# divortio/divortio-lz4

Hardware: NVIDIA B200
Metric: lz4_block_roundtrip_throughput (higher is better)
Workload: dtype u8

## Files before the change

### divortio-lz4_b200/csrc/api_ctx.inc

```
namespace {

constexpr int kWarpsFresh16 = 7;
constexpr int kWarpsGeneric32 = 3;
constexpr int kWarpsDecode = 8;
constexpr int kJdGroupEvent = 112;
constexpr int kGtabRegions = 5;
constexpr uint32_t kMaxSplitBlocks = 1u << 20;

struct Buf {
    void *p = nullptr;
    size_t cap = 0;
};

class CopyPool {
  public:
    explicit CopyPool(int threads) {
        for (int i = 0; i < threads; ++i) workers_.emplace_back([this] { run(); });
    }
    ~CopyPool() {
        { std::lock_guard<std::mutex> g(m_); stop_ = true; }
        cv_.notify_all();
        for (std::thread &t : workers_) t.join();
    }
    void copy(void *dst, const void *src, size_t n) {
// ... 42 lines not shown
    std::vector<std::thread> workers_;
    std::mutex m_;
    std::condition_variable cv_, cv_done_;
    bool stop_ = false;
    uint64_t gen_ = 0;
    uint8_t *dst_ = nullptr;
    const uint8_t *src_ = nullptr;
    size_t n_ = 0, piece_ = 0, parts_ = 0, done_ = 0;
    std::atomic<size_t> next_{0};
};
constexpr int kSumSlots = 32;
constexpr int kStageSlots = 4;
constexpr size_t kStageBytes = 16u << 20;

}

struct dlz4_ctx {
    int device = 0;
    int sm_count = 0;
    cudaStream_t stream = nullptr, side = nullptr, copy_in = nullptr, copy_out = nullptr;
    cudaStream_t lanes[4] = {};
    uint64_t chunk_bytes = 64ull << 20;
    int n_lanes = 3;
    cudaEvent_t evp[128] = {};
    cudaEvent_t ev0 = nullptr, ev1 = nullptr, ev_side = nullptr, ev_fork = nullptr;
    uint32_t *d_counter = nullptr;
    uint32_t *d_land = nullptr;
    uint32_t *h_one = nullptr;
    uint64_t seg_overlap_min_bytes = 64ull << 20;
    uint32_t *d_hash = nullptr;
    uint64_t *d_total = nullptr;
    int32_t *d_table = nullptr;
    int split = 1;
    int pw = 2;
    int pw_sleep = 200;
    int pw_lead = 7;
    Buf rec;
    uint32_t *d_nrec = nullptr;
    int hybrid = 1;
    int hy_grid = 0;
    int hy_active = 0;
    uint16_t *d_gtabs = nullptr;
    Buf work, comp, seg, out, meta, aux, pin;
    std::string last_error;
    uint64_t frame_pipe_min_bytes = 32ull << 20;
    uint64_t jump_min_bytes = 256ull << 10;
    uint64_t seg_min_bytes = 256ull << 10;
    uint32_t seg_jobs = 0, seg_reruns = 0, seg_rounds = 0;
    uint64_t launches = 0;
    float last_ms = 0.f;
    int64_t k_seg_kib = -1, k_seg_warm_kib = -1, k_seg_unit_kib = -1;
    int k_seg_group = -1, k_seg_no_chase = 0, k_jd_unit_mib = 0, k_jd_serial_scan = 0, k_jd_no_overlap = 0, k_debug = 0;
    CopyPool *pool = nullptr;
    int copy_threads = 0;
    uint8_t *stage[kStageSlots] = {};
    cudaEvent_t stage_ev[kStageSlots] = {};
    bool stage_busy[kStageSlots] = {};
    cudaStream_t sum_stream[kSumSlots] = {};
    uint32_t *h_sum = nullptr;
    int probe = 0;
    cudaEvent_t evq[3] = {};
    const uint8_t *res_in = nullptr, *res_out = nullptr;
    uint64_t res_in_len = 0, res_out_len = 0, res_body_len = 0;
};

namespace {

// ... 123 lines not shown
```

### divortio-lz4_b200/csrc/api_launch.inc

```
int compress_segmented(dlz4_ctx *ctx, const uint8_t *d_work, int64_t start, int64_t total, int64_t B, uint32_t n, bool linked,
                       const int32_t *init_table, uint8_t *d_comp, const uint64_t *d_coff, uint32_t *d_clen, cudaStream_t st,
                       int32_t *final_table = nullptr, const uint32_t *landed = nullptr, int32_t land_origin = 0,
                       uint32_t land_shift = 0);

int launch_compress(dlz4_ctx *ctx, const uint8_t *src, const uint64_t *src_off, const uint32_t *src_len, uint32_t n,
                    uint32_t max_len, const uint8_t *prefix, uint32_t prefix_len, const int32_t *init_table, uint8_t *dst,
                    const uint64_t *dst_off, uint32_t *comp_len, cudaStream_t st, uint32_t *counter = nullptr, bool dense = false) {
    if (n == 0) return DLZ4_OK;
    if (!counter) counter = ctx->d_counter;
    CK(cudaMemsetAsync(counter, 0, sizeof(uint32_t), st));
    if (init_table == nullptr) { prefix = nullptr; prefix_len = 0; }
    if (max_len <= 65536 && prefix_len == 0 && init_table == nullptr && ctx->split && n <= kMaxSplitBlocks) {
        const size_t region = (size_t)(counter - ctx->d_counter) % kGtabRegions;
        const uint64_t rstride = (uint64_t)max_len / 4 + 2;
        const size_t region_bytes = (((size_t)n * rstride * 8) * 9 / 8 + 255) & ~(size_t)255;
        if (ctx->rec.cap < region_bytes * kGtabRegions + 256) {
            CK(cudaDeviceSynchronize());
            CKS(reserve(ctx, ctx->rec, std::max(region_bytes, (size_t)ctx->rec.cap / kGtabRegions) * kGtabRegions));
        }
        const size_t per_region = ((ctx->rec.cap - 256) / kGtabRegions) & ~(size_t)255;
        uint64_t *recs = (uint64_t *)((uint8_t *)ctx->rec.p + region * per_region);
        uint32_t *nrec = ctx->d_nrec + region * (size_t)kMaxSplitBlocks;
        if (ctx->probe) CK(cudaEventRecord(ctx->evq[0], st));
        if (ctx->pw) {
            const int grid = (int)std::min<uint64_t>(n, (uint64_t)ctx->sm_count);
            const uint32_t lead = (uint32_t)ctx->pw_lead, ns = (uint32_t)ctx->pw_sleep;
            const size_t sm = (size_t)kPwChains * kPwChainBytes;
            if (ctx->pw == 2)
                k_parse_pw<2><<<grid, kPwChains * 3 * 32, sm, st>>>(src, src_off, src_len, n, recs, rstride, nrec, counter, lead, ns);
            else
                k_parse_pw<3><<<grid, kPwChains * 4 * 32, sm, st>>>(src, src_off, src_len, n, recs, rstride, nrec, counter, lead, ns);
        } else
        {
            const int grid = (int)std::min<uint64_t>((n + kWarpsFresh16 - 1) / kWarpsFresh16, (uint64_t)ctx->sm_count);
            k_parse_fresh16<kWarpsFresh16><<<grid, kWarpsFresh16 * 32, kWarpsFresh16 * kHashEntries * 2, st>>>(
                src, src_off, src_len, n, recs, rstride, nrec, counter);
        }
        if (ctx->probe) CK(cudaEventRecord(ctx->evq[1], st));
        CK(cudaMemsetAsync(counter, 0, sizeof(uint32_t), st));
        const int egrid = (int)std::min<uint64_t>((n + kWarpsDecode - 1) / kWarpsDecode, (uint64_t)ctx->sm_count * 8);
        k_encode_blocks<kWarpsDecode><<<egrid, kWarpsDecode * 32, 0, st>>>(src, src_off, src_len, n, recs, rstride, nrec, dst, dst_off,
                                                                            comp_len, counter);
        if (ctx->probe) CK(cudaEventRecord(ctx->evq[2], st));
        ctx->launches++;
    } else if (max_len <= 65536 && prefix_len == 0 && init_table == nullptr && ctx->hybrid) {
        const size_t region = (size_t)(counter - ctx->d_counter) % kGtabRegions;
        const int grid = (int)std::min<uint64_t>(dense ? (n + kHyWarps - 1) / kHyWarps : n, (uint64_t)ctx->hy_grid);
        uint32_t active = dense ? (uint32_t)kHyWarps : (uint32_t)std::min<uint64_t>((n + grid - 1) / grid, (uint64_t)kHyWarps);
        if (ctx->hy_active) active = std::min<uint32_t>(active, (uint32_t)ctx->hy_active);
        k_compress_fresh16h<<<grid, kHyWarps * 32, kHySmemBytes, st>>>(
            src, src_off, src_len, n, dst, dst_off, comp_len, counter,
            ctx->d_gtabs + region * (size_t)ctx->hy_grid * kHyGlWarps * kHashEntries, active);
    } else if (max_len <= 4096 && prefix_len > 0 && init_table != nullptr && ctx->hybrid && prefix_len < 0x7FFF0000u) {
        const size_t region = (size_t)(counter - ctx->d_counter) % kGtabRegions;
        const int grid = (int)std::min<uint64_t>(dense ? (n + kHyWarps - 1) / kHyWarps : n, (uint64_t)ctx->hy_grid);
        const uint32_t active = dense ? (uint32_t)kHyWarps : (uint32_t)std::min<uint64_t>((n + grid - 1) / grid, (uint64_t)kHyWarps);
        k_compress_overlay<<<grid, kHyWarps * 32, kHySmemBytes, st>>>(
            src, src_off, src_len, n, prefix, prefix_len, init_table, dst, dst_off, comp_len, counter,
            ctx->d_gtabs + region * (size_t)ctx->hy_grid * kHyGlWarps * kHashEntries, active);
    } else {
        if (max_len > 65536 && prefix_len == 0 && init_table == nullptr && n <= 65536) {
            std::vector<uint64_t> off(n);
            std::vector<uint32_t> len(n);
            CK(cudaMemcpyAsync(off.data(), src_off, (size_t)n * 8, cudaMemcpyDeviceToHost, st));
// ... 57 lines not shown
```

### divortio-lz4_b200/csrc/api_lifecycle.inc

```
int dlz4_init(int device, dlz4_ctx **out) {
    if (!out) return DLZ4_E_INVALID_ARG;
    *out = nullptr;
    dlz4_ctx *ctx = new dlz4_ctx();
    ctx->device = device;
    *out = ctx;
    int count = 0;
    CK(cudaGetDeviceCount(&count));
    if (device < 0 || device >= count) { ctx->last_error = "no such CUDA device"; return DLZ4_E_CUDA; }
    CK(cudaSetDevice(device));
    cudaDeviceProp prop;
    CK(cudaGetDeviceProperties(&prop, device));
    ctx->sm_count = prop.multiProcessorCount;
    CK(cudaStreamCreateWithFlags(&ctx->stream, cudaStreamNonBlocking));
    CK(cudaStreamCreateWithFlags(&ctx->side, cudaStreamNonBlocking));
    CK(cudaStreamCreateWithFlags(&ctx->copy_in, cudaStreamNonBlocking));
    CK(cudaStreamCreateWithFlags(&ctx->copy_out, cudaStreamNonBlocking));
    for (cudaEvent_t &e : ctx->evp) CK(cudaEventCreateWithFlags(&e, cudaEventDisableTiming));
    CK(cudaEventCreate(&ctx->ev0));
    CK(cudaEventCreate(&ctx->ev1));
    for (cudaEvent_t &e : ctx->evq) CK(cudaEventCreate(&e));
    CK(cudaEventCreateWithFlags(&ctx->ev_side, cudaEventDisableTiming));
    CK(cudaEventCreateWithFlags(&ctx->ev_fork, cudaEventDisableTiming));
    for (cudaStream_t &l : ctx->lanes) CK(cudaStreamCreateWithFlags(&l, cudaStreamNonBlocking));
    if (const char *e = getenv("DLZ4_SEG_KIB")) ctx->k_seg_kib = std::max(0, atoi(e));
    if (const char *e = getenv("DLZ4_SEG_WARM_KIB")) ctx->k_seg_warm_kib = std::max(0, atoi(e));
    if (const char *e = getenv("DLZ4_SEG_UNIT_KIB")) ctx->k_seg_unit_kib = std::max(0, atoi(e));
    if (const char *e = getenv("DLZ4_SEG_GROUP")) ctx->k_seg_group = std::max(0, atoi(e));
    ctx->k_seg_no_chase = getenv("DLZ4_SEG_NO_CHASE") != nullptr;
    if (const char *e = getenv("DLZ4_JD_UNIT_MIB")) ctx->k_jd_unit_mib = std::max(1, atoi(e));
    ctx->k_jd_serial_scan = getenv("DLZ4_JD_SERIAL_SCAN") != nullptr;
    ctx->k_jd_no_overlap = getenv("DLZ4_JD_NO_OVERLAP") != nullptr;
    ctx->k_debug = getenv("DLZ4_DEBUG") != nullptr;
    if (const char *e = getenv("DLZ4_CHUNK_MIB")) ctx->chunk_bytes = (uint64_t)std::max(1, atoi(e)) << 20;
    if (const char *e = getenv("DLZ4_LANES")) ctx->n_lanes = std::min(4, std::max(1, atoi(e)));
    if (const char *e = getenv("DLZ4_COPY_THREADS")) ctx->copy_threads = std::min(64, std::max(1, atoi(e)));
    CK(cudaMalloc(&ctx->d_counter, 64));
    CK(cudaMalloc(&ctx->d_land, kLandFlags * 4));
    CK(cudaMallocHost(&ctx->h_one, 64));
    *ctx->h_one = 1u;
    if (const char *e = getenv("DLZ4_SEG_OVERLAP_MIN_MIB")) ctx->seg_overlap_min_bytes = (uint64_t)atoll(e) << 20;
    CK(cudaMalloc(&ctx->d_hash, 64));
    CK(cudaMalloc(&ctx->d_total, 64));
    CK(cudaMalloc(&ctx->d_table, kHashEntries * sizeof(int32_t)));
    if (const char *e = getenv("DLZ4_SEG_MIN_KIB")) ctx->seg_min_bytes = (uint64_t)atoll(e) << 10;
    if (const char *e = getenv("DLZ4_JUMP_MIN_KIB")) ctx->jump_min_bytes = (uint64_t)atoll(e) << 10;
    if (const char *e = getenv("DLZ4_SPLIT")) ctx->split = atoi(e) != 0;
    if (const char *e = getenv("DLZ4_PW")) ctx->pw = std::max(0, std::min(3, atoi(e)));
    if (const char *e = getenv("DLZ4_PW_SLEEP")) ctx->pw_sleep = std::max(0, atoi(e));
    if (const char *e = getenv("DLZ4_PW_LEAD")) ctx->pw_lead = std::max(3, std::min(kPwWin - 1, atoi(e)));
    if (const char *e = getenv("DLZ4_HYBRID")) ctx->hybrid = atoi(e) != 0;
    ctx->hy_grid = ctx->sm_count * kHyCtasPerSm;
    if (const char *e = getenv("DLZ4_HY_ACTIVE")) ctx->hy_active = std::max(0, std::min(kHyWarps, atoi(e)));
    CK(cudaMalloc(&ctx->d_gtabs, (size_t)kGtabRegions * ctx->hy_grid * kHyGlWarps * kHashEntries * 2));
    CK(cudaMalloc(&ctx->d_nrec, (size_t)kGtabRegions * kMaxSplitBlocks * 4));
    CK(cudaFuncSetAttribute(k_parse_fresh16<kWarpsFresh16>, cudaFuncAttributeMaxDynamicSharedMemorySize, kWarpsFresh16 * kHashEntries * 2));
    CK(cudaFuncSetAttribute(k_parse_pw<2>, cudaFuncAttributeMaxDynamicSharedMemorySize, kPwChains * kPwChainBytes));
    CK(cudaFuncSetAttribute(k_parse_pw<3>, cudaFuncAttributeMaxDynamicSharedMemorySize, kPwChains * kPwChainBytes));
    CK(cudaFuncSetAttribute(k_compress_fresh16h, cudaFuncAttributeMaxDynamicSharedMemorySize, kHySmemBytes));
    CK(cudaFuncSetAttribute(k_compress_overlay, cudaFuncAttributeMaxDynamicSharedMemorySize, kHySmemBytes));
    CK(cudaFuncSetAttribute(k_compress_segments, cudaFuncAttributeMaxDynamicSharedMemorySize, kSegSmemBytes));
    CK(cudaFuncSetAttribute(k_compress_generic32<kWarpsGeneric32>, cudaFuncAttributeMaxDynamicSharedMemorySize,
                            kWarpsGeneric32 * (kHashEntries * 4 + kRingBytes)));
    CK(cudaFuncSetAttribute(k_compress_chain, cudaFuncAttributeMaxDynamicSharedMemorySize, kHashEntries * 4 + kRingBytes));
    return DLZ4_OK;
}

void dlz4_shutdown(dlz4_ctx *ctx) {
    if (!ctx) return;
    cudaSetDevice(ctx->device);
    if (ctx->stream) cudaStreamSynchronize(ctx->stream);
    if (ctx->side) cudaStreamSynchronize(ctx->side);
    for (Buf *b : {&ctx->work, &ctx->comp, &ctx->seg, &ctx->out, &ctx->meta, &ctx->aux})
        if (b->p) cudaFree(b->p);
    if (ctx->pin.p) cudaFreeHost(ctx->pin.p);
    if (ctx->d_counter) cudaFree(ctx->d_counter);
    if (ctx->d_land) cudaFree(ctx->d_land);
    if (ctx->h_one) cudaFreeHost(ctx->h_one);
    if (ctx->d_hash) cudaFree(ctx->d_hash);
    if (ctx->d_total) cudaFree(ctx->d_total);
    if (ctx->d_table) cudaFree(ctx->d_table);
    if (ctx->d_gtabs) cudaFree(ctx->d_gtabs);
    if (ctx->d_nrec) cudaFree(ctx->d_nrec);
    if (ctx->rec.p) cudaFree(ctx->rec.p);
    delete ctx->pool;
    for (cudaStream_t s : ctx->sum_stream) if (s) { cudaStreamSynchronize(s); cudaStreamDestroy(s); }
    if (ctx->h_sum) cudaFreeHost(ctx->h_sum);
    for (int i = 0; i < kStageSlots; ++i) {
        if (ctx->stage[i]) cudaFreeHost(ctx->stage[i]);
        if (ctx->stage_ev[i]) cudaEventDestroy(ctx->stage_ev[i]);
    }
// ... 88 lines not shown
```

### divortio-lz4_b200/csrc/dlz4_pw.cuh

```cuda
#pragma once

namespace dlz4 {

constexpr int kPwChains = 6;
constexpr int kPwWin = 14;
constexpr int kPwRingBytes = kPwWin * 32 * 12;
constexpr int kPwCtl = 64;
constexpr int kPwChainBytes = kHashEntries * 2 + kPwRingBytes + kPwCtl;
constexpr uint32_t kPwRingSmc = 160u;
constexpr uint32_t kPwDone = 0x80000000u, kPwSparse = 0x40000000u;
constexpr bool kPwPrefetch = true;
#ifndef DLZ4_PW_CAP
#define DLZ4_PW_CAP 32
#endif
constexpr uint32_t kPwCap = DLZ4_PW_CAP;

struct PwCtl {
    volatile uint32_t w_pos;
    volatile uint32_t block;
};

__device__ __forceinline__ void pw_bar(uint32_t id, uint32_t nthreads) {
    asm volatile("bar.sync %0, %1;" ::"r"(id), "r"(nthreads) : "memory");
}
__device__ __forceinline__ uint32_t pw_lds(const uint32_t *p) {
    uint32_t v;
    asm volatile("ld.volatile.shared.u32 %0, [%1];" : "=r"(v) : "r"((uint32_t)__cvta_generic_to_shared(p)) : "memory");
    return v;
}
__device__ __forceinline__ void pw_sts(uint32_t *p, const uint32_t v) {
    asm volatile("st.volatile.shared.u32 [%0], %1;" ::"r"((uint32_t)__cvta_generic_to_shared(p)), "r"(v) : "memory");
}
__device__ __forceinline__ void pw_prefetch(const void *p) { asm volatile("prefetch.global.L1 [%0];" ::"l"(p)); }
__device__ __forceinline__ uint32_t pw_slot(const uint32_t p) {
    const uint32_t w = p >> 5;
    const uint32_t ws = w - (uint32_t)kPwWin * ((w * 74899u) >> 20);
    return ws * 96u + (p & 31u);
}
__device__ __forceinline__ uint32_t pw_resolve(const uint32_t ml, const uint32_t lane, uint32_t &exitp) {
    uint32_t n = ml == kPwCap ? 255u : lane + (ml ? ml : 1u);
    uint32_t m = 1u << lane;
#pragma unroll
    for (int r = 0; r < 5; ++r) {
        const uint32_t mj = __shfl_sync(FULL, m, n), nj = __shfl_sync(FULL, n, n);
        if (n < 32u) { m |= mj; n = nj; }
    }
    exitp = n;
    return m;
}

__device__ __forceinline__ uint32_t pw_extend(const uint8_t *__restrict__ base, int32_t s0, int32_t m0, int32_t eb,
                                              int32_t matchLimit, uint32_t lane) {
    const int32_t back = s0 - m0;
    auto round4 = [&](int32_t e0, uint32_t &res) -> bool {
        const int32_t q = s0 + e0 + 4 * (int32_t)lane;
        int32_t nv = matchLimit - q;
        nv = nv > 4 ? 4 : nv;
        int32_t eq = 0;
        if (nv > 0) {
            const uint32_t x = ld32u(base + q) ^ ld32u(base + q - back);
            const int32_t e = x ? ((__ffs(x) - 1) >> 3) : 4;
            eq = e < nv ? e : nv;
        }
        const uint32_t stop = __ballot_sync(FULL, eq < 4);
        if (!stop) return false;
        const int l = __ffs(stop) - 1;
        res = (uint32_t)(e0 + 4 * l + __shfl_sync(FULL, eq, l));
        return true;
    };
    uint32_t res = 0;
// ... 9 lines not shown
    const uint32_t cmis = (uint32_t)(reinterpret_cast<uintptr_t>(cb) & 15u);
    const uint32_t wsel = cmis >> 2, bsh = (cmis & 3u) * 8u;
    for (;; eb += 2048) {
        uint32_t eqb[4];
#pragma unroll
        for (int u = 0; u < 4; ++u) {
            const int32_t q = s0 + eb + 512 * u + 16 * (int32_t)lane;
            int32_t nv = matchLimit - q;
            nv = nv > 16 ? 16 : nv;
            eqb[u] = 0;
            if (nv > 0) {
                const uint4 a = __ldg(reinterpret_cast<const uint4 *>(base + q));
                const uint4 *cp = reinterpret_cast<const uint4 *>(base + q - back - (int32_t)cmis);
                const uint4 c0 = __ldg(cp), c1 = __ldg(cp + 1);
                uint32_t v[8] = {c0.x, c0.y, c0.z, c0.w, c1.x, c1.y, c1.z, c1.w};
                uint32_t t[5];
#pragma unroll
                for (int i = 0; i < 5; ++i) t[i] = wsel == 0 ? v[i] : wsel == 1 ? v[i + 1] : wsel == 2 ? v[i + 2] : v[i + 3];
                const uint32_t x0 = a.x ^ __funnelshift_r(t[0], t[1], bsh), x1 = a.y ^ __funnelshift_r(t[1], t[2], bsh);
                const uint32_t x2 = a.z ^ __funnelshift_r(t[2], t[3], bsh), x3 = a.w ^ __funnelshift_r(t[3], t[4], bsh);
                uint32_t e = x0 ? ((uint32_t)(__ffs(x0) - 1) >> 3) : x1 ? 4u + ((uint32_t)(__ffs(x1) - 1) >> 3)
                           : x2 ? 8u + ((uint32_t)(__ffs(x2) - 1) >> 3) : x3 ? 12u + ((uint32_t)(__ffs(x3) - 1) >> 3) : 16u;
                eqb[u] = e < (uint32_t)nv ? e : (uint32_t)nv;
            }
        }
#pragma unroll
        for (int u = 0; u < 4; ++u) {
            const uint32_t stop = __ballot_sync(FULL, eqb[u] < 16u);
            if (stop) { const int l = __ffs(stop) - 1; return (uint32_t)(eb + 512 * u + 16 * l) + __shfl_sync(FULL, eqb[u], l); }
        }
    }
}

constexpr uint32_t kPwGenMask = 0x7FFu;

__device__ __forceinline__ uint32_t pw_count32(const uint4 &q0, const uint4 &q1, const uint4 &q2, const uint32_t cs, const uint32_t *Sw) {
    uint32_t v[12] = {q0.x, q0.y, q0.z, q0.w, q1.x, q1.y, q1.z, q1.w, q2.x, q2.y, q2.z, q2.w};
    const bool s8 = (cs & 8u) != 0, s4 = (cs & 4u) != 0;
#pragma unroll
    for (int k = 0; k < 10; ++k) v[k] = s8 ? v[k + 2] : v[k];
#pragma unroll
    for (int k = 0; k < 9; ++k) v[k] = s4 ? v[k + 1] : v[k];
    const uint32_t csh = (cs & 3u) * 8u;
    uint32_t x[8];
#pragma unroll
    for (int k = 0; k < 8; ++k) x[k] = Sw[k] ^ __funnelshift_r(v[k], v[k + 1], csh);
    const bool h4 = (x[0] | x[1] | x[2] | x[3]) == 0u;
    const uint32_t y0 = h4 ? x[4] : x[0], y1 = h4 ? x[5] : x[1], y2 = h4 ? x[6] : x[2], y3 = h4 ? x[7] : x[3];
    const bool h2 = (y0 | y1) == 0u;
    const uint32_t z0 = h2 ? y2 : y0, z1 = h2 ? y3 : y1;
    const bool h1 = z0 == 0u;
    const uint32_t zz = h1 ? z1 : z0;
    return (h4 ? 16u : 0u) + (h2 ? 8u : 0u) + (h1 ? 4u : 0u) + (zz ? ((uint32_t)(__ffs(zz) - 1) >> 3) : 4u);
}

__device__ __forceinline__ void pw_produce2(const uint8_t *__restrict__ base, const uint32_t k, const bool two, const uint16_t *tab,
                                            uint32_t *ring, const uint32_t lane) {
    const uint32_t pa = 32u * k + lane, pb = pa + 32u;
    const uintptr_t ba = reinterpret_cast<uintptr_t>(base);
    const uint32_t a = (uint32_t)(ba & 3u) + pa;
    const uint32_t *wp = reinterpret_cast<const uint32_t *>(ba & ~(uintptr_t)3) + (a >> 2);
    const uint32_t sh = (a & 3u) * 8u;
    uint32_t w[17];
#pragma unroll
    for (int i = 0; i < 9; ++i) w[i] = __ldg(wp + i);
#pragma unroll
    for (int i = 9; i < 17; ++i) w[i] = two ? __ldg(wp + i) : 0u;
    uint32_t S[16];
#pragma unroll
    for (int i = 0; i < 16; ++i) S[i] = __funnelshift_r(w[i], w[i + 1], sh);
    const uint32_t ha = (S[0] * 2654435761u) >> 18, hb = (S[8] * 2654435761u) >> 18;
    const uint32_t seena = *reinterpret_cast<const volatile uint16_t *>(tab + ha);
    const uint32_t seenb = *reinterpret_cast<const volatile uint16_t *>(tab + hb);
    const bool oka = seena != pa, okb = two && seenb != pb;
    const uint32_t la = oka ? seena : pa, lb = okb ? seenb : pa;
    const uint32_t csa = ((uint32_t)(ba & 15u) + la) & 15u, csb = ((uint32_t)(ba & 15u) + lb) & 15u;
    const uint4 *cqa = reinterpret_cast<const uint4 *>(base + la - csa), *cqb = reinterpret_cast<const uint4 *>(base + lb - csb);
    const uint4 qa0 = __ldg(cqa), qa1 = __ldg(cqa + 1), qa2 = __ldg(cqa + 2);
    const uint4 qb0 = __ldg(cqb), qb1 = __ldg(cqb + 1), qb2 = __ldg(cqb + 2);
    if (kPwPrefetch) {
        pw_prefetch(cqa + 4);
        if (two) { pw_prefetch(cqb + 4); pw_prefetch(wp + 24); }
    }
    const uint32_t va = wide_verify(qa0, qa1, qa2, csa, S), vb = wide_verify(qb0, qb1, qb2, csb, S + 8);
    uint32_t mla = oka ? va : 0u, mlb = okb ? vb : 0u;
    if (kPwCap > 32u && __any_sync(FULL, mla == 32u || mlb == 32u)) {
        if (mla == 32u) {
            const uint4 q3 = __ldg(cqa + 3), q4 = __ldg(cqa + 4);
            mla += two ? pw_count32(qa2, q3, q4, csa, S + 8) : 0u;
        }
        if (mlb == 32u) {
            uint32_t w2[9], S2[8];
#pragma unroll
            for (int i = 0; i < 9; ++i) w2[i] = __ldg(wp + 16 + i);
#pragma unroll
            for (int i = 0; i < 8; ++i) S2[i] = __funnelshift_r(w2[i], w2[i + 1], sh);
            const uint4 q3 = __ldg(cqb + 3), q4 = __ldg(cqb + 4);
            mlb += pw_count32(qb2, q3, q4, csb, S2);
        }
    }
    if (kPwCap > 32u && !two && mla == 32u) {
        uint32_t w2[9], S2[8];
#pragma unroll
        for (int i = 0; i < 9; ++i) w2[i] = __ldg(wp + 8 + i);
#pragma unroll
        for (int i = 0; i < 8; ++i) S2[i] = __funnelshift_r(w2[i], w2[i + 1], sh);
        const uint4 q3 = __ldg(cqa + 3), q4 = __ldg(cqa + 4);
        mla += pw_count32(qa2, q3, q4, csa, S2);
    }
    uint32_t exa, exb;
    const uint32_t pma = pw_resolve(mla, lane, exa), pmb = pw_resolve(mlb, lane, exb);
    const uint32_t loa = ha | (mla << 14) | (((k + 1u) & kPwGenMask) << 21);
    uint32_t *const sa = ring + pw_slot(pa), *const sb = ring + pw_slot(pb);
    pw_sts(sa + 32, seena | (exa << 16));
    pw_sts(sa + 64, pma);
    if (two) {
        pw_sts(sb + 32, seenb | (exb << 16));
        pw_sts(sb + 64, pmb);
    }
    __threadfence_block();
    pw_sts(sa, loa);
    if (two) pw_sts(sb, hb | (mlb << 14) | (((k + 2u) & kPwGenMask) << 21));
}

template <int kNP>
__device__ __forceinline__ void pw_producer(const uint8_t *__restrict__ base, const uint32_t nwin, const uint32_t lead,
                                            const uint32_t j, const uint16_t *tab, uint32_t *ring, PwCtl *ctl, const uint32_t lane,
                                            const uint32_t full_ns) {
    uint32_t k = 2u * j;
    PT_DECL
    for (;;) {
        const uint32_t wpos = ctl->w_pos;
        if (wpos & kPwDone) break;
        if (wpos & kPwSparse) { __nanosleep(1024); PT_MARK(8) continue; }
        const uint32_t wk = wpos >> 5;
        if (k + 1u < wk) k += (wk - k - 2u + 2u * (uint32_t)kNP) / (2u * (uint32_t)kNP) * (2u * (uint32_t)kNP);
        if (k >= nwin) { __nanosleep(1024); PT_MARK(8) continue; }
        if (k + 1u >= wk + lead) { __nanosleep(full_ns); PT_MARK(7) continue; }
        if (kPwPrefetch && lane < 2u && k + 2u * (uint32_t)kNP < nwin) pw_prefetch(base + 32u * (k + 2u * (uint32_t)kNP) + 128u * lane);
        pw_produce2(base, k, k + 1u < nwin, tab, ring, lane);
        PT_MARK(6) PT_COUNT(13, 1)
        k += 2u * (uint32_t)kNP;
    }
    PT_FLUSH
}

__device__ __forceinline__ uint32_t pw_walker(const uint8_t *__restrict__ base, const int32_t len, const uint32_t nwin, uint16_t *tab,
                                              const uint32_t *ring, PwCtl *ctl, uint64_t *__restrict__ rec, const uint32_t lane) {
    const uint32_t lt = (1u << lane) - 1u;
    const int32_t sEnd = len;
    const int32_t mflimit = sEnd - 12;
    const int32_t matchLimit = sEnd - 5;
    const int32_t plimit = (int32_t)(32u * nwin);
    const int32_t rlimit = plimit < mflimit ? plimit : mflimit;
    int32_t sIndex = 0;
    uint32_t smc = 67;
    uint32_t nrec = 0;
    uint32_t pub = 0;
    const SrcFlat S{base};
    Tab16 T{tab, 0};
    uint2 *const rec2 = reinterpret_cast<uint2 *>(rec);
    PT_DECL

    while (sIndex < mflimit) {
        if (smc <= 96u && (sIndex | 31) < rlimit) {
            const uint32_t s = (uint32_t)sIndex, wbase = s & ~31u, sl = s & 31u;
            if (pub != wbase) { pub = wbase; if (lane == 0) ctl->w_pos = wbase; }
            const uint32_t p = wbase + lane;
            const uint32_t want = ((p >> 5) + 1u) & kPwGenMask;
            const uint32_t *slot = ring + pw_slot(p);
            uint32_t ex;
            PT_MARK(14)
            for (;;) {
                ex = pw_lds(slot);
                if (__all_sync(FULL, (ex >> 21) == want)) break;
                __nanosleep(32);
                PT_COUNT(15, 1)
            }
            PT_MARK(1)
            const uint32_t ey = pw_lds(slot + 32);
            const uint32_t PM = pw_lds(slot + 64 + sl - lane), exitp = pw_lds(slot + 32 + sl - lane) >> 16;
            const uint32_t seen = ey & 0xFFFFu;
            const uint32_t h = ex & 0x3FFFu, ml = (ex >> 14) & 127u;
            const uint32_t cur = tab[h];
            const uint32_t claim = __ballot_sync(FULL, ml != 0u);
            const bool probed = (PM >> lane) & 1u;
            const uint32_t tag = p & 0xFFFFu;
            __syncwarp();
            if (probed) tab[h] = (uint16_t)tag;
            __syncwarp();
            const uint32_t r = probed ? (uint32_t)tab[h] : tag;
            const uint32_t bad = __ballot_sync(FULL, probed && (r != tag || cur != seen));
            if (!bad) {
                const uint32_t HM = PM & claim;
                const uint32_t nh = (uint32_t)__popc(HM);
                if (((HM >> lane) & 1u) && ml != kPwCap) rec2[nrec + (uint32_t)__popc(HM & lt)] = rec_pack(p, ml, p - cur);
                if (exitp == 255u) {
                    const uint32_t c = 31u - (uint32_t)__clz(PM);
                    const uint32_t pc = wbase + c, curc = __shfl_sync(FULL, cur, c);
                    const uint32_t mlx = pw_extend(base, (int32_t)pc, (int32_t)curc, (int32_t)kPwCap, matchLimit, lane);
                    if (lane == 0) rec2[nrec + nh - 1u] = rec_pack(pc, mlx, pc - curc);
                    sIndex = (int32_t)(pc + mlx);
                    smc = 67u;
                } else {
                    sIndex = (int32_t)(wbase + exitp);
                    if (HM) smc = 67u + (uint32_t)__popc(PM & ~((2u << (31 - __clz(HM))) - 1u));
                    else smc += (uint32_t)__popc(PM);
                }
                nrec += nh;
                PT_MARK(0) PT_COUNT(9, 1)
                continue;
            }
            const uint32_t inv = (probed && r != tag) ? min(tag, r) : 0xFFFFFFFFu;
            const uint32_t cutpos = __reduce_min_sync(FULL, inv);
// ... 3 lines not shown
            if (probed && lane >= Bl) tab[h] = (uint16_t)cur;
            __syncwarp();
            if (probed && lane < Bl) tab[h] = (uint16_t)tag;
            __syncwarp();
            const uint32_t keep = PM & below, HMk = keep & claim;
            if ((HMk >> lane) & 1u) rec2[nrec + (uint32_t)__popc(HMk & lt)] = rec_pack(p, ml, p - cur);
            nrec += (uint32_t)__popc(HMk);
            if (HMk) smc = 67u + (uint32_t)__popc(keep & ~((2u << (31 - __clz(HMk))) - 1u));
            else smc += (uint32_t)__popc(keep);
            sIndex = (int32_t)(wbase + (uint32_t)__ffs(PM & ~below) - 1u);
            const uint32_t hx = __shfl_sync(FULL, h, (uint32_t)sIndex - wbase);
            const uint32_t cand = tab[hx];
            __syncwarp();
            if (lane == 0) tab[hx] = (uint16_t)sIndex;
            __syncwarp();
            uint32_t mlx = 0;
            if (cand != (uint32_t)sIndex) mlx = pw_extend(base, sIndex, (int32_t)cand, 0, matchLimit, lane);
            if (mlx >= 4u) {
                if (lane == 0) rec2[nrec] = rec_pack((uint32_t)sIndex, mlx, (uint32_t)sIndex - cand);
                ++nrec;
                sIndex += (int32_t)mlx;
                smc = 67u;
            } else {
                sIndex += (int32_t)(smc >> 6);
                ++smc;
            }
            PT_MARK(4) PT_COUNT(10, 1)
            continue;
        }
        if (smc <= kPwRingSmc && sIndex < rlimit) {
            const uint32_t bs = skip_sum(smc);
            const int32_t p = sIndex + (int32_t)(skip_sum(smc + lane) - bs);
            const bool valid = p < rlimit;
            if (pub != (uint32_t)sIndex) { pub = (uint32_t)sIndex; if (lane == 0) ctl->w_pos = pub; }
            const uint32_t *slot = ring + pw_slot((uint32_t)p);
            const uint32_t want = (((uint32_t)p >> 5) + 1u) & kPwGenMask;
            uint32_t lo;
            for (;;) {
                lo = pw_lds(slot);
                const bool ready = !valid || ((lo >> 21) == want);
                if (__all_sync(FULL, ready)) break;
                __nanosleep(20);
            }
            const uint32_t seen = pw_lds(slot + 32) & 0xFFFFu;
            const uint32_t h = lo & 0x3FFFu, ml = (lo >> 14) & 127u;
            const uint32_t cur = tab[h];
            const uint32_t claim = __ballot_sync(FULL, valid && ml != 0u);
            const uint32_t f = claim ? (uint32_t)__ffs(claim) - 1u : 32u;
            const bool active = valid && lane <= f;
            const uint32_t tag = (uint32_t)p & 0xFFFFu;
            __syncwarp();
            if (active) tab[h] = (uint16_t)tag;
            __syncwarp();
            const uint32_t r = active ? (uint32_t)tab[h] : tag;
            const uint32_t bad = __ballot_sync(FULL, active && (r != tag || cur != seen));
            if (!bad) {
                if (claim) {
                    const int32_t pf = sIndex + (int32_t)(skip_sum(smc + f) - bs);
                    const uint32_t curf = __shfl_sync(FULL, cur, f);
                    uint32_t mlf = __shfl_sync(FULL, ml, f);
                    if (mlf == kPwCap) mlf = pw_extend(base, pf, (int32_t)curf, (int32_t)kPwCap, matchLimit, lane);
                    if (lane == 0) rec2[nrec] = rec_pack((uint32_t)pf, mlf, (uint32_t)pf - curf);
                    ++nrec;
                    sIndex = pf + (int32_t)mlf;
                    smc = 67u;
                } else {
                    const uint32_t nv = (uint32_t)__popc(__ballot_sync(FULL, valid));
                    sIndex += (int32_t)(skip_sum(smc + nv) - bs);
                    smc += nv;
                }
                PT_MARK(2) PT_COUNT(11, 1)
                continue;
            }
            const uint32_t inv = (active && r != tag) ? min((uint32_t)p, r) : 0xFFFFFFFFu;
            const uint32_t cutpos = __reduce_min_sync(FULL, inv);
            const uint32_t grp = __ballot_sync(FULL, active && (uint32_t)p <= cutpos);
            const uint32_t stale = __ballot_sync(FULL, active && cur != seen);
            const uint32_t c = min((uint32_t)__popc(grp), stale ? (uint32_t)__ffs(stale) - 1u : 32u);
            if (active && lane >= c) tab[h] = (uint16_t)cur;
            __syncwarp();
            if (active && lane < c) tab[h] = (uint16_t)tag;
            __syncwarp();
            if (c != 0u) {
                sIndex += (int32_t)(skip_sum(smc + c) - bs);
                smc += c;
                PT_MARK(2) PT_COUNT(11, 1)
                continue;
            }
            const uint32_t h0 = __shfl_sync(FULL, h, 0);
            const uint32_t cand = tab[h0];
            __syncwarp();
            if (lane == 0) tab[h0] = (uint16_t)sIndex;
            __syncwarp();
            uint32_t ml0 = 0;
            if (cand != (uint32_t)sIndex) ml0 = pw_extend(base, sIndex, (int32_t)cand, 0, matchLimit, lane);
            if (ml0 >= 4u) {
                if (lane == 0) rec2[nrec] = rec_pack((uint32_t)sIndex, ml0, (uint32_t)sIndex - cand);
                ++nrec;
                sIndex += (int32_t)ml0;
                smc = 67u;
            } else {
                sIndex += (int32_t)(smc >> 6);
                ++smc;
            }
            PT_MARK(2) PT_COUNT(11, 1)
            continue;
        }

        if (smc > kPwRingSmc && sIndex < rlimit) {
            const uint32_t v = (uint32_t)sIndex | kPwSparse;
            if (pub != v) { pub = v; if (lane == 0) ctl->w_pos = pub; }
        }
        const uint32_t base_sum = skip_sum(smc);
        const int32_t p = sIndex + (int32_t)(skip_sum(smc + lane) - base_sum);
        const bool valid = p < mflimit;
        uint32_t seq = 0, h = 0x10000u + lane;
        int32_t cand = -1;
        if (valid) {
            seq = S.ld32(p);
            h = (seq * 2654435761u) >> 18;
            cand = T.get(h);
        }
        const uint32_t same = __match_any_sync(FULL, h);
        const uint32_t prev = same & lt;
        const int j = prev ? 31 - __clz(prev) : (int)lane;
        const int32_t pj = __shfl_sync(FULL, p, j);
        const uint32_t sj = __shfl_sync(FULL, seq, j);
        uint32_t cseq = sj;
        if (prev) cand = pj;
        const bool ok = valid && cand >= 0 && cand != p && (((uint32_t)(p - cand)) >> 16) == 0;
        if (ok && !prev) cseq = S.ld32(cand);
        const bool hit = ok && cseq == seq;
        const uint32_t hits = __ballot_sync(FULL, hit);
        const uint32_t vmask = __ballot_sync(FULL, valid);
        const int hl = __ffs(hits) - 1;
        const uint32_t commit = hits ? ((2u << hl) - 1u) : vmask;
        if (((commit >> lane) & 1u) && ((same & commit) >> lane) == 1u) T.put(h, p);
        __syncwarp();
        if (!hits) {
            if (vmask != FULL) break;
            sIndex += (int32_t)(skip_sum(smc + 32u) - base_sum);
            smc += 32u;
            PT_MARK(3) PT_COUNT(12, 1)
            continue;
        }
        const int32_t s0 = __shfl_sync(FULL, p, hl);
        const int32_t m0 = __shfl_sync(FULL, cand, hl);
        smc = 67;
        const uint32_t ml = pw_extend(base, s0, m0, 4, matchLimit, lane);
        if (lane == 0) rec2[nrec] = rec_pack((uint32_t)s0, ml, (uint32_t)(s0 - m0));
        ++nrec;
        sIndex = s0 + (int32_t)ml;
        PT_MARK(3) PT_COUNT(12, 1)
    }
    PT_MARK(5)
    PT_FLUSH
    return nrec;
}

template <int kNP>
__global__ void __launch_bounds__(kPwChains * (1 + kNP) * 32, 1)
k_parse_pw(const uint8_t *__restrict__ src, const uint64_t *__restrict__ src_off, const uint32_t *__restrict__ src_len,
           uint32_t nblocks, uint64_t *__restrict__ rec_base, uint64_t rec_stride ,
           uint32_t *__restrict__ nrec_out, uint32_t *counter, uint32_t lead,
           uint32_t full_ns ) {
    extern __shared__ __align__(16) uint8_t smem[];
    constexpr uint32_t kRoles = 1 + kNP;
    constexpr uint32_t kTeam = kRoles * 32;
    const uint32_t lane = lane_id(), warp = threadIdx.x >> 5;
    const uint32_t chain = warp / kRoles, role = warp % kRoles;
    const uint32_t tid = threadIdx.x - chain * kTeam;
    uint8_t *const cb = smem + (size_t)chain * kPwChainBytes;
    uint16_t *const tab = reinterpret_cast<uint16_t *>(cb);
    uint32_t *const ring = reinterpret_cast<uint32_t *>(cb + kHashEntries * 2);
    PwCtl *const ctl = reinterpret_cast<PwCtl *>(cb + kHashEntries * 2 + kPwRingBytes);
    const uint32_t bar = 1u + chain;
    uint32_t first = chain * gridDim.x + blockIdx.x;
    const uint32_t qbase = gridDim.x * (uint32_t)kPwChains;
    bool have_first = true;
    for (;;) {
        pw_bar(bar, kTeam);
        if (role == 0 && lane == 0) {
            uint32_t b;
            if (have_first) b = first; else b = qbase + atomicAdd(counter, 1u);
            ctl->block = b < nblocks ? b : 0xFFFFFFFFu;
            ctl->w_pos = 0u;
        }
        have_first = false;
        pw_bar(bar, kTeam);
        const uint32_t b = ctl->block;
        if (b == 0xFFFFFFFFu) return;
        const uint32_t len = src_len[b];
        if (len > 65536u) {
            if (role == 0 && lane == 0) nrec_out[b] = 0xFFFFFFFFu;
            continue;
        }
        {
            uint4 *z = reinterpret_cast<uint4 *>(cb);
            for (uint32_t i = tid; i < (kHashEntries * 2 + kPwRingBytes) / 16; i += kTeam) z[i] = make_uint4(0, 0, 0, 0);
        }
        pw_bar(bar, kTeam);
        const uint8_t *base = src + src_off[b];
        uint64_t *const rec = rec_base + (uint64_t)b * rec_stride;
        const uint32_t nwin = len >= 112u ? (len - 111u) / 32u + 1u : 0u;
        if (role == 0) {
            const uint32_t n = pw_walker(base, (int32_t)len, nwin, tab, ring, ctl, rec, lane);
            if (lane == 0) {
                nrec_out[b] = n;
                ctl->w_pos = kPwDone;
            }
        } else {
            pw_producer<kNP>(base, nwin, lead, role - 1u, tab, ring, ctl, lane, full_ns);
        }
    }
}

}
```

Baseline: 75.24.

## Move parse-walker producer ring from shared memory into tensor memory

```diff
diff --git a/divortio-lz4_b200/csrc/api_ctx.inc b/divortio-lz4_b200/csrc/api_ctx.inc
--- a/divortio-lz4_b200/csrc/api_ctx.inc
+++ b/divortio-lz4_b200/csrc/api_ctx.inc
@@ -98,7 +98,7 @@
     uint64_t *d_total = nullptr;
     int32_t *d_table = nullptr;
     int split = 1;
-    int pw = 2;
+    bool pw = true;
     int pw_sleep = 200;
     int pw_lead = 7;
     Buf rec;
diff --git a/divortio-lz4_b200/csrc/api_launch.inc b/divortio-lz4_b200/csrc/api_launch.inc
--- a/divortio-lz4_b200/csrc/api_launch.inc
+++ b/divortio-lz4_b200/csrc/api_launch.inc
@@ -25,11 +25,7 @@
         if (ctx->pw) {
             const int grid = (int)std::min<uint64_t>(n, (uint64_t)ctx->sm_count);
             const uint32_t lead = (uint32_t)ctx->pw_lead, ns = (uint32_t)ctx->pw_sleep;
-            const size_t sm = (size_t)kPwChains * kPwChainBytes;
-            if (ctx->pw == 2)
-                k_parse_pw<2><<<grid, kPwChains * 3 * 32, sm, st>>>(src, src_off, src_len, n, recs, rstride, nrec, counter, lead, ns);
-            else
-                k_parse_pw<3><<<grid, kPwChains * 4 * 32, sm, st>>>(src, src_off, src_len, n, recs, rstride, nrec, counter, lead, ns);
+            k_parse_pw<<<grid, kPwThreads, kPwSmemBytes, st>>>(src, src_off, src_len, n, recs, rstride, nrec, counter, lead, ns);
         } else
         {
             const int grid = (int)std::min<uint64_t>((n + kWarpsFresh16 - 1) / kWarpsFresh16, (uint64_t)ctx->sm_count);
diff --git a/divortio-lz4_b200/csrc/api_lifecycle.inc b/divortio-lz4_b200/csrc/api_lifecycle.inc
--- a/divortio-lz4_b200/csrc/api_lifecycle.inc
+++ b/divortio-lz4_b200/csrc/api_lifecycle.inc
@@ -45,7 +45,7 @@
     if (const char *e = getenv("DLZ4_SEG_MIN_KIB")) ctx->seg_min_bytes = (uint64_t)atoll(e) << 10;
     if (const char *e = getenv("DLZ4_JUMP_MIN_KIB")) ctx->jump_min_bytes = (uint64_t)atoll(e) << 10;
     if (const char *e = getenv("DLZ4_SPLIT")) ctx->split = atoi(e) != 0;
-    if (const char *e = getenv("DLZ4_PW")) ctx->pw = std::max(0, std::min(3, atoi(e)));
+    if (const char *e = getenv("DLZ4_PW")) ctx->pw = atoi(e) != 0;
     if (const char *e = getenv("DLZ4_PW_SLEEP")) ctx->pw_sleep = std::max(0, atoi(e));
     if (const char *e = getenv("DLZ4_PW_LEAD")) ctx->pw_lead = std::max(3, std::min(kPwWin - 1, atoi(e)));
     if (const char *e = getenv("DLZ4_HYBRID")) ctx->hybrid = atoi(e) != 0;
@@ -54,8 +54,7 @@
     CK(cudaMalloc(&ctx->d_gtabs, (size_t)kGtabRegions * ctx->hy_grid * kHyGlWarps * kHashEntries * 2));
     CK(cudaMalloc(&ctx->d_nrec, (size_t)kGtabRegions * kMaxSplitBlocks * 4));
     CK(cudaFuncSetAttribute(k_parse_fresh16<kWarpsFresh16>, cudaFuncAttributeMaxDynamicSharedMemorySize, kWarpsFresh16 * kHashEntries * 2));
-    CK(cudaFuncSetAttribute(k_parse_pw<2>, cudaFuncAttributeMaxDynamicSharedMemorySize, kPwChains * kPwChainBytes));
-    CK(cudaFuncSetAttribute(k_parse_pw<3>, cudaFuncAttributeMaxDynamicSharedMemorySize, kPwChains * kPwChainBytes));
+    CK(cudaFuncSetAttribute(k_parse_pw, cudaFuncAttributeMaxDynamicSharedMemorySize, kPwSmemBytes));
     CK(cudaFuncSetAttribute(k_compress_fresh16h, cudaFuncAttributeMaxDynamicSharedMemorySize, kHySmemBytes));
     CK(cudaFuncSetAttribute(k_compress_overlay, cudaFuncAttributeMaxDynamicSharedMemorySize, kHySmemBytes));
     CK(cudaFuncSetAttribute(k_compress_segments, cudaFuncAttributeMaxDynamicSharedMemorySize, kSegSmemBytes));
diff --git a/divortio-lz4_b200/csrc/dlz4_pw.cuh b/divortio-lz4_b200/csrc/dlz4_pw.cuh
--- a/divortio-lz4_b200/csrc/dlz4_pw.cuh
+++ b/divortio-lz4_b200/csrc/dlz4_pw.cuh
@@ -2,11 +2,14 @@
 
 namespace dlz4 {
 
-constexpr int kPwChains = 6;
+constexpr int kPwChains = 7;
+constexpr int kPwProducers = 2;
+constexpr int kPwThreads = 8 * (1 + kPwProducers) * 32;
 constexpr int kPwWin = 14;
-constexpr int kPwRingBytes = kPwWin * 32 * 12;
+constexpr uint32_t kPwTmemCols = 128;
 constexpr int kPwCtl = 64;
-constexpr int kPwChainBytes = kHashEntries * 2 + kPwRingBytes + kPwCtl;
+constexpr int kPwChainBytes = kHashEntries * 2 + kPwCtl;
+constexpr int kPwSmemBytes = kPwChains * kPwChainBytes + 16;
 constexpr uint32_t kPwRingSmc = 160u;
 constexpr uint32_t kPwDone = 0x80000000u, kPwSparse = 0x40000000u;
 constexpr bool kPwPrefetch = true;
@@ -16,26 +19,49 @@
 constexpr uint32_t kPwCap = DLZ4_PW_CAP;
 
 struct PwCtl {
-    volatile uint32_t w_pos;
+    uint32_t w_pos;
     volatile uint32_t block;
+    uint32_t ready[kPwWin];
 };
+static_assert(sizeof(PwCtl) <= kPwCtl, "PwCtl");
 
 __device__ __forceinline__ void pw_bar(uint32_t id, uint32_t nthreads) {
     asm volatile("bar.sync %0, %1;" ::"r"(id), "r"(nthreads) : "memory");
 }
-__device__ __forceinline__ uint32_t pw_lds(const uint32_t *p) {
+__device__ __forceinline__ uint32_t pw_ld_acquire(const uint32_t *p) {
     uint32_t v;
-    asm volatile("ld.volatile.shared.u32 %0, [%1];" : "=r"(v) : "r"((uint32_t)__cvta_generic_to_shared(p)) : "memory");
+    asm volatile("ld.acquire.cta.shared.u32 %0, [%1];" : "=r"(v) : "r"((uint32_t)__cvta_generic_to_shared(p)) : "memory");
     return v;
 }
-__device__ __forceinline__ void pw_sts(uint32_t *p, const uint32_t v) {
-    asm volatile("st.volatile.shared.u32 [%0], %1;" ::"r"((uint32_t)__cvta_generic_to_shared(p)), "r"(v) : "memory");
+__device__ __forceinline__ void pw_st_release(uint32_t *p, const uint32_t v) {
+    asm volatile("st.release.cta.shared.u32 [%0], %1;" ::"r"((uint32_t)__cvta_generic_to_shared(p)), "r"(v) : "memory");
+}
+__device__ __forceinline__ void pw_st_release2(uint32_t *p, const uint32_t v0, const uint32_t v1) {
+    asm volatile("st.release.cta.shared.v2.u32 [%0], {%1, %2};" ::"r"((uint32_t)__cvta_generic_to_shared(p)), "r"(v0), "r"(v1) : "memory");
 }
 __device__ __forceinline__ void pw_prefetch(const void *p) { asm volatile("prefetch.global.L1 [%0];" ::"l"(p)); }
-__device__ __forceinline__ uint32_t pw_slot(const uint32_t p) {
-    const uint32_t w = p >> 5;
-    const uint32_t ws = w - (uint32_t)kPwWin * ((w * 74899u) >> 20);
-    return ws * 96u + (p & 31u);
+__device__ __forceinline__ void tm_fence_before() { asm volatile("tcgen05.fence::before_thread_sync;" ::: "memory"); }
+__device__ __forceinline__ void tm_fence_after() { asm volatile("tcgen05.fence::after_thread_sync;" ::: "memory"); }
+__device__ __forceinline__ void tm_st8(const uint32_t t, const uint32_t x0, const uint32_t y0, const uint32_t z0, const uint32_t x1,
+                                       const uint32_t y1, const uint32_t z1) {
+    asm volatile("tcgen05.st.sync.aligned.32x32b.x8.b32 [%0], {%1, %2, %3, %3, %4, %5, %6, %6};\n\t"
+                 "tcgen05.wait::st.sync.aligned;" ::"r"(t), "r"(x0), "r"(y0), "r"(z0), "r"(x1), "r"(y1), "r"(z1) : "memory");
+}
+__device__ __forceinline__ void tm_ld4(const uint32_t t, uint32_t &x, uint32_t &y, uint32_t &z) {
+    uint32_t u;
+    asm volatile("tcgen05.ld.sync.aligned.32x32b.x4.b32 {%0, %1, %2, %3}, [%4];\n\t"
+                 "tcgen05.wait::ld.sync.aligned;\n\t"
+                 "tcgen05.fence::before_thread_sync;" : "=r"(x), "=r"(y), "=r"(z), "=r"(u) : "r"(t) : "memory");
+}
+__device__ __forceinline__ void tm_ld2(const uint32_t t, uint32_t &x, uint32_t &y) {
+    asm volatile("tcgen05.ld.sync.aligned.32x32b.x2.b32 {%0, %1}, [%2];\n\t"
+                 "tcgen05.wait::ld.sync.aligned;\n\t"
+                 "tcgen05.fence::before_thread_sync;" : "=r"(x), "=r"(y) : "r"(t) : "memory");
+}
+__device__ __forceinline__ uint32_t pw_ws(const uint32_t w) { return w - (uint32_t)kPwWin * ((w * 74899u) >> 20); }
+__device__ __forceinline__ void pw_wait_ready(const PwCtl *ctl, const uint32_t ws, const uint32_t w, const uint32_t ns) {
+    while (!__all_sync(FULL, pw_ld_acquire(ctl->ready + ws) == w + 1u)) __nanosleep(ns);
+    tm_fence_after();
 }
 __device__ __forceinline__ uint32_t pw_resolve(const uint32_t ml, const uint32_t lane, uint32_t &exitp) {
     uint32_t n = ml == kPwCap ? 255u : lane + (ml ? ml : 1u);
@@ -111,7 +137,6 @@
     }
 }
 
-constexpr uint32_t kPwGenMask = 0x7FFu;
 
 __device__ __forceinline__ uint32_t pw_count32(const uint4 &q0, const uint4 &q1, const uint4 &q2, const uint32_t cs, const uint32_t *Sw) {
     uint32_t v[12] = {q0.x, q0.y, q0.z, q0.w, q1.x, q1.y, q1.z, q1.w, q2.x, q2.y, q2.z, q2.w};
@@ -134,7 +159,7 @@
 }
 
 __device__ __forceinline__ void pw_produce2(const uint8_t *__restrict__ base, const uint32_t k, const bool two, const uint16_t *tab,
-                                            uint32_t *ring, const uint32_t lane) {
+                                            const uint32_t tcol, PwCtl *ctl, const uint32_t lane) {
     const uint32_t pa = 32u * k + lane, pb = pa + 32u;
     const uintptr_t ba = reinterpret_cast<uintptr_t>(base);
     const uint32_t a = (uint32_t)(ba & 3u) + pa;
@@ -189,27 +214,23 @@
     }
     uint32_t exa, exb;
     const uint32_t pma = pw_resolve(mla, lane, exa), pmb = pw_resolve(mlb, lane, exb);
-    const uint32_t loa = ha | (mla << 14) | (((k + 1u) & kPwGenMask) << 21);
-    uint32_t *const sa = ring + pw_slot(pa), *const sb = ring + pw_slot(pb);
-    pw_sts(sa + 32, seena | (exa << 16));
-    pw_sts(sa + 64, pma);
-    if (two) {
-        pw_sts(sb + 32, seenb | (exb << 16));
-        pw_sts(sb + 64, pmb);
-    }
-    __threadfence_block();
-    pw_sts(sa, loa);
-    if (two) pw_sts(sb, hb | (mlb << 14) | (((k + 2u) & kPwGenMask) << 21));
-}
-
-template <int kNP>
+    const uint32_t ws = pw_ws(k);
+    __syncwarp();
+    tm_fence_after();
+    tm_st8(tcol + 4u * ws, ha | (mla << 14), seena | (exa << 16), pma, hb | (mlb << 14), seenb | (exb << 16), pmb);
+    tm_fence_before();
+    if (two) pw_st_release2(ctl->ready + ws, k + 1u, k + 2u);
+    else pw_st_release(ctl->ready + ws, k + 1u);
+}
+
 __device__ __forceinline__ void pw_producer(const uint8_t *__restrict__ base, const uint32_t nwin, const uint32_t lead,
-                                            const uint32_t j, const uint16_t *tab, uint32_t *ring, PwCtl *ctl, const uint32_t lane,
+                                            const uint32_t j, const uint16_t *tab, const uint32_t tcol, PwCtl *ctl, const uint32_t lane,
                                             const uint32_t full_ns) {
+    constexpr int kNP = kPwProducers;
     uint32_t k = 2u * j;
     PT_DECL
     for (;;) {
-        const uint32_t wpos = ctl->w_pos;
+        const uint32_t wpos = pw_ld_acquire(&ctl->w_pos);
         if (wpos & kPwDone) break;
         if (wpos & kPwSparse) { __nanosleep(1024); PT_MARK(8) continue; }
         const uint32_t wk = wpos >> 5;
@@ -217,7 +238,7 @@
         if (k >= nwin) { __nanosleep(1024); PT_MARK(8) continue; }
         if (k + 1u >= wk + lead) { __nanosleep(full_ns); PT_MARK(7) continue; }
         if (kPwPrefetch && lane < 2u && k + 2u * (uint32_t)kNP < nwin) pw_prefetch(base + 32u * (k + 2u * (uint32_t)kNP) + 128u * lane);
-        pw_produce2(base, k, k + 1u < nwin, tab, ring, lane);
+        pw_produce2(base, k, k + 1u < nwin, tab, tcol, ctl, lane);
         PT_MARK(6) PT_COUNT(13, 1)
         k += 2u * (uint32_t)kNP;
     }
@@ -225,7 +246,7 @@
 }
 
 __device__ __forceinline__ uint32_t pw_walker(const uint8_t *__restrict__ base, const int32_t len, const uint32_t nwin, uint16_t *tab,
-                                              const uint32_t *ring, PwCtl *ctl, uint64_t *__restrict__ rec, const uint32_t lane) {
+                                              const uint32_t tcol, PwCtl *ctl, uint64_t *__restrict__ rec, const uint32_t lane) {
     const uint32_t lt = (1u << lane) - 1u;
     const int32_t sEnd = len;
     const int32_t mflimit = sEnd - 12;
@@ -244,21 +265,19 @@
     while (sIndex < mflimit) {
         if (smc <= 96u && (sIndex | 31) < rlimit) {
             const uint32_t s = (uint32_t)sIndex, wbase = s & ~31u, sl = s & 31u;
-            if (pub != wbase) { pub = wbase; if (lane == 0) ctl->w_pos = wbase; }
+            if (pub != wbase) { pub = wbase; if (lane == 0) pw_st_release(&ctl->w_pos, wbase); }
             const uint32_t p = wbase + lane;
-            const uint32_t want = ((p >> 5) + 1u) & kPwGenMask;
-            const uint32_t *slot = ring + pw_slot(p);
-            uint32_t ex;
+            const uint32_t w = wbase >> 5, ws = pw_ws(w);
             PT_MARK(14)
-            for (;;) {
-                ex = pw_lds(slot);
-                if (__all_sync(FULL, (ex >> 21) == want)) break;
+            while (!__all_sync(FULL, pw_ld_acquire(ctl->ready + ws) == w + 1u)) {
                 __nanosleep(32);
                 PT_COUNT(15, 1)
             }
+            tm_fence_after();
+            uint32_t ex, ey, ez;
+            tm_ld4(tcol + 4u * ws, ex, ey, ez);
             PT_MARK(1)
-            const uint32_t ey = pw_lds(slot + 32);
-            const uint32_t PM = pw_lds(slot + 64 + sl - lane), exitp = pw_lds(slot + 32 + sl - lane) >> 16;
+            const uint32_t PM = __shfl_sync(FULL, ez, sl), exitp = __shfl_sync(FULL, ey, sl) >> 16;
             const uint32_t seen = ey & 0xFFFFu;
             const uint32_t h = ex & 0x3FFFu, ml = (ex >> 14) & 127u;
             const uint32_t cur = tab[h];
@@ -328,17 +347,20 @@
             const uint32_t bs = skip_sum(smc);
             const int32_t p = sIndex + (int32_t)(skip_sum(smc + lane) - bs);
             const bool valid = p < rlimit;
-            if (pub != (uint32_t)sIndex) { pub = (uint32_t)sIndex; if (lane == 0) ctl->w_pos = pub; }
-            const uint32_t *slot = ring + pw_slot((uint32_t)p);
-            const uint32_t want = (((uint32_t)p >> 5) + 1u) & kPwGenMask;
-            uint32_t lo;
-            for (;;) {
-                lo = pw_lds(slot);
-                const bool ready = !valid || ((lo >> 21) == want);
-                if (__all_sync(FULL, ready)) break;
-                __nanosleep(20);
-            }
-            const uint32_t seen = pw_lds(slot + 32) & 0xFFFFu;
+            if (pub != (uint32_t)sIndex) { pub = (uint32_t)sIndex; if (lane == 0) pw_st_release(&ctl->w_pos, pub); }
+            const uint32_t w0 = (uint32_t)sIndex >> 5;
+            const uint32_t wl = (uint32_t)min(__shfl_sync(FULL, p, 31), rlimit - 1) >> 5;
+            uint32_t lo = 0, ye = 0;
+            for (uint32_t w = w0; w <= wl; ++w) {
+                const uint32_t ws = pw_ws(w);
+                pw_wait_ready(ctl, ws, w, 20);
+                uint32_t xw, yw;
+                tm_ld2(tcol + 4u * ws, xw, yw);
+                xw = __shfl_sync(FULL, xw, (uint32_t)p & 31u);
+                yw = __shfl_sync(FULL, yw, (uint32_t)p & 31u);
+                if (((uint32_t)p >> 5) == w) { lo = xw; ye = yw; }
+            }
+            const uint32_t seen = ye & 0xFFFFu;
             const uint32_t h = lo & 0x3FFFu, ml = (lo >> 14) & 127u;
             const uint32_t cur = tab[h];
             const uint32_t claim = __ballot_sync(FULL, valid && ml != 0u);
@@ -405,7 +427,7 @@
 
         if (smc > kPwRingSmc && sIndex < rlimit) {
             const uint32_t v = (uint32_t)sIndex | kPwSparse;
-            if (pub != v) { pub = v; if (lane == 0) ctl->w_pos = pub; }
+            if (pub != v) { pub = v; if (lane == 0) pw_st_release(&ctl->w_pos, pub); }
         }
         const uint32_t base_sum = skip_sum(smc);
         const int32_t p = sIndex + (int32_t)(skip_sum(smc + lane) - base_sum);
@@ -454,61 +476,79 @@
     return nrec;
 }
 
-template <int kNP>
-__global__ void __launch_bounds__(kPwChains * (1 + kNP) * 32, 1)
+__global__ void __launch_bounds__(kPwThreads, 1)
 k_parse_pw(const uint8_t *__restrict__ src, const uint64_t *__restrict__ src_off, const uint32_t *__restrict__ src_len,
            uint32_t nblocks, uint64_t *__restrict__ rec_base, uint64_t rec_stride ,
            uint32_t *__restrict__ nrec_out, uint32_t *counter, uint32_t lead,
            uint32_t full_ns ) {
     extern __shared__ __align__(16) uint8_t smem[];
-    constexpr uint32_t kRoles = 1 + kNP;
+    constexpr uint32_t kRoles = 1 + kPwProducers;
     constexpr uint32_t kTeam = kRoles * 32;
     const uint32_t lane = lane_id(), warp = threadIdx.x >> 5;
-    const uint32_t chain = warp / kRoles, role = warp % kRoles;
-    const uint32_t tid = threadIdx.x - chain * kTeam;
-    uint8_t *const cb = smem + (size_t)chain * kPwChainBytes;
-    uint16_t *const tab = reinterpret_cast<uint16_t *>(cb);
-    uint32_t *const ring = reinterpret_cast<uint32_t *>(cb + kHashEntries * 2);
-    PwCtl *const ctl = reinterpret_cast<PwCtl *>(cb + kHashEntries * 2 + kPwRingBytes);
-    const uint32_t bar = 1u + chain;
-    uint32_t first = chain * gridDim.x + blockIdx.x;
-    const uint32_t qbase = gridDim.x * (uint32_t)kPwChains;
-    bool have_first = true;
-    for (;;) {
-        pw_bar(bar, kTeam);
-        if (role == 0 && lane == 0) {
-            uint32_t b;
-            if (have_first) b = first; else b = qbase + atomicAdd(counter, 1u);
-            ctl->block = b < nblocks ? b : 0xFFFFFFFFu;
-            ctl->w_pos = 0u;
-        }
-        have_first = false;
-        pw_bar(bar, kTeam);
-        const uint32_t b = ctl->block;
-        if (b == 0xFFFFFFFFu) return;
-        const uint32_t len = src_len[b];
-        if (len > 65536u) {
-            if (role == 0 && lane == 0) nrec_out[b] = 0xFFFFFFFFu;
-            continue;
-        }
-        {
-            uint4 *z = reinterpret_cast<uint4 *>(cb);
-            for (uint32_t i = tid; i < (kHashEntries * 2 + kPwRingBytes) / 16; i += kTeam) z[i] = make_uint4(0, 0, 0, 0);
-        }
-        pw_bar(bar, kTeam);
-        const uint8_t *base = src + src_off[b];
-        uint64_t *const rec = rec_base + (uint64_t)b * rec_stride;
-        const uint32_t nwin = len >= 112u ? (len - 111u) / 32u + 1u : 0u;
-        if (role == 0) {
-            const uint32_t n = pw_walker(base, (int32_t)len, nwin, tab, ring, ctl, rec, lane);
-            if (lane == 0) {
-                nrec_out[b] = n;
-                ctl->w_pos = kPwDone;
-            }
-        } else {
-            pw_producer<kNP>(base, nwin, lead, role - 1u, tab, ring, ctl, lane, full_ns);
-        }
-    }
-}
-
-}
+    const uint32_t quarter = warp & 3u, tslot = (warp >> 2) / kRoles, role = (warp >> 2) % kRoles;
+    const uint32_t chain = quarter + 4u * tslot;
+    uint32_t *const taddr_smem = reinterpret_cast<uint32_t *>(smem + kPwChains * kPwChainBytes);
+    if (warp == 0) {
+        asm volatile("tcgen05.alloc.cta_group::1.sync.aligned.shared::cta.b32 [%0], %1;\n\t"
+                     "tcgen05.relinquish_alloc_permit.cta_group::1.sync.aligned;"
+                     ::"r"((uint32_t)__cvta_generic_to_shared(taddr_smem)), "r"(kPwTmemCols) : "memory");
+    }
+    tm_fence_before();
+    __syncthreads();
+    tm_fence_after();
+    const uint32_t taddr = *taddr_smem;
+    const uint32_t tcol = taddr + ((32u * quarter) << 16) + tslot * (uint32_t)(kPwWin * 4);
+    if (chain < (uint32_t)kPwChains) {
+        const uint32_t tid = role * 32u + lane;
+        uint8_t *const cb = smem + (size_t)chain * kPwChainBytes;
+        uint16_t *const tab = reinterpret_cast<uint16_t *>(cb);
+        PwCtl *const ctl = reinterpret_cast<PwCtl *>(cb + kHashEntries * 2);
+        const uint32_t bar = 1u + chain;
+        uint32_t first = chain * gridDim.x + blockIdx.x;
+        const uint32_t qbase = gridDim.x * (uint32_t)kPwChains;
+        bool have_first = true;
+        for (;;) {
+            pw_bar(bar, kTeam);
+            if (role == 0 && lane == 0) {
+                uint32_t b;
+                if (have_first) b = first; else b = qbase + atomicAdd(counter, 1u);
+                ctl->block = b < nblocks ? b : 0xFFFFFFFFu;
+                ctl->w_pos = 0u;
+            }
+            have_first = false;
+            pw_bar(bar, kTeam);
+            const uint32_t b = ctl->block;
+            if (b == 0xFFFFFFFFu) break;
+            const uint32_t len = src_len[b];
+            if (len > 65536u) {
+                if (role == 0 && lane == 0) nrec_out[b] = 0xFFFFFFFFu;
+                continue;
+            }
+            {
+                uint4 *z = reinterpret_cast<uint4 *>(cb);
+                for (uint32_t i = tid; i < kHashEntries * 2 / 16; i += kTeam) z[i] = make_uint4(0, 0, 0, 0);
+                if (tid < (uint32_t)kPwWin) ctl->ready[tid] = 0u;
+            }
+            pw_bar(bar, kTeam);
+            const uint8_t *base = src + src_off[b];
+            uint64_t *const rec = rec_base + (uint64_t)b * rec_stride;
+            const uint32_t nwin = len >= 112u ? (len - 111u) / 32u + 1u : 0u;
+            if (role == 0) {
+                const uint32_t n = pw_walker(base, (int32_t)len, nwin, tab, tcol, ctl, rec, lane);
+                if (lane == 0) {
+                    nrec_out[b] = n;
+                    pw_st_release(&ctl->w_pos, kPwDone);
+                }
+            } else {
+                pw_producer(base, nwin, lead, role - 1u, tab, tcol, ctl, lane, full_ns);
+            }
+        }
+    }
+    tm_fence_before();
+    __syncthreads();
+    tm_fence_after();
+    if (warp == 0)
+        asm volatile("tcgen05.dealloc.cta_group::1.sync.aligned.b32 %0, %1;" ::"r"(taddr), "r"(kPwTmemCols) : "memory");
+}
+
+}
```

After: 78.52 (median of 6 runs). 4.4% higher.
